# Victarry/Image-Generation-models

Measured on AMD Instinct MI355X. Metric: ddpm_cifar10_32x32_train_images_per_sec, higher is better.
Workload: dtype bf16; 1 GPU; DDPM CIFAR-10 32x32, UNet 128/1-2-4, T=1000 (BASELINE configs[1]): train step B=128/GPU + hipGraph denoise step B=64; per_gpu_batch=128, global_batch=128, parallelism=dp1, step_launch=hipGraph replay, denoise_batch=64, rccl_ranks=1, state_finite=True, matmul=bf16 MFMA, fp32 accumulate

## Files before the change

### image-generation-models_amd/csrc/norm_act.hip

```cpp
#include <stdlib.h>
#include "common.h"

#ifndef MI_GN_UB0
#define MI_GN_UB0 4
#endif
#ifndef MI_GN_PD
#define MI_GN_PD 2
#endif
#ifndef MI_GN_ABL
#define MI_GN_ABL 0
#endif
#ifndef MI_GN_FULL16
#define MI_GN_FULL16 0
#endif
#ifndef MI_GN_WAVES
#define MI_GN_WAVES 4
#endif

namespace {

template <int VEC> struct V;
template <> struct V<4> {
    float v[4];
    __device__ static V load(const float* p) { float4 t = *reinterpret_cast<const float4*>(p); return V{{t.x, t.y, t.z, t.w}}; }
// ... 577 lines not shown
    }
}

template <bool DY16, int LPX, int MAXV>
__global__ __launch_bounds__(256) void chan_ln_bwd_kernel(const LnArgs a) {
    MI_PRIO_UP();
    constexpr int PPW = 64 / LPX;
    __shared__ float red[2][4][LPX * MAXV * 4];
    const int l = threadIdx.x & 63, w = threadIdx.x >> 6, lp = l % LPX;
    const int nq = a.C / 4;
    float4 ag[MAXV], ab[MAXV], gg[MAXV];
#pragma unroll
    for (int k = 0; k < MAXV; ++k) {
        ag[k] = ab[k] = make_float4(0.f, 0.f, 0.f, 0.f);
        int q = lp + LPX * k;
        gg[k] = (q < nq) ? *reinterpret_cast<const float4*>(a.g + 4 * q) : make_float4(0.f, 0.f, 0.f, 0.f);
    }
    for (int m0 = (blockIdx.x * 4 + w) * PPW; m0 < a.M; m0 += gridDim.x * 4 * PPW) {
        const int m = min(m0 + l / LPX, a.M - 1);
        const float live = m0 + l / LPX < a.M ? 1.f : 0.f;
        const float* xp = a.x + (size_t)m * a.ldx;
        float4 c[MAXV], d[MAXV];
        float s = 0.f;
#pragma unroll
        for (int k = 0; k < MAXV; ++k) {
            int q = lp + LPX * k;
            if (q < nq) {
                c[k] = *reinterpret_cast<const float4*>(xp + 4 * q);
                const V<4> dv = vload<4, DY16>(a.dy, (size_t)m * a.lddy + 4 * q);
                d[k] = make_float4(dv.v[0] * live, dv.v[1] * live, dv.v[2] * live, dv.v[3] * live);
                s += c[k].x + c[k].y + c[k].z + c[k].w;
            }
        }
        const float mean = group_sum<LPX>(s) / (float)a.C;
        float s2 = 0.f, sh = 0.f, sS = 0.f;
#pragma unroll
        for (int k = 0; k < MAXV; ++k) {
            if (lp + LPX * k < nq) {
                c[k].x -= mean; c[k].y -= mean; c[k].z -= mean; c[k].w -= mean;
                s2 += c[k].x * c[k].x + c[k].y * c[k].y + c[k].z * c[k].z + c[k].w * c[k].w;
                float h0 = d[k].x * gg[k].x, h1 = d[k].y * gg[k].y, h2 = d[k].z * gg[k].z, h3 = d[k].w * gg[k].w;
                sh += h0 + h1 + h2 + h3;
                sS += h0 * c[k].x + h1 * c[k].y + h2 * c[k].z + h3 * c[k].w;
            }
        }
        const float var = group_sum<LPX>(s2) / (float)a.C;
        const float mh = group_sum<LPX>(sh) / (float)a.C;
        const float S = group_sum<LPX>(sS);
        const float sigma = sqrtf(var);
        const float inv = 1.0f / (sigma + a.eps);
        const float k2 = sigma > 0.f ? inv * inv * S / (sigma * (float)a.C) : 0.f;
        float* op = a.dx + (size_t)m * a.lddx;
        const float* ip = a.dx_in + (size_t)m * a.lddx_in;
#pragma unroll
        for (int k = 0; k < MAXV; ++k) {
            int q = lp + LPX * k;
            if (q < nq) {
                float4 o;
                o.x = inv * (d[k].x * gg[k].x - mh) - k2 * c[k].x;
                o.y = inv * (d[k].y * gg[k].y - mh) - k2 * c[k].y;
                o.z = inv * (d[k].z * gg[k].z - mh) - k2 * c[k].z;
                o.w = inv * (d[k].w * gg[k].w - mh) - k2 * c[k].w;
                if (live != 0.f) {
                    if (a.accumulate) {
                        float4 prev = *reinterpret_cast<const float4*>(ip + 4 * q);
                        o.x += prev.x; o.y += prev.y; o.z += prev.z; o.w += prev.w;
                    }
                    *reinterpret_cast<float4*>(op + 4 * q) = o;
                }
                ag[k].x += d[k].x * c[k].x * inv; ag[k].y += d[k].y * c[k].y * inv;
                ag[k].z += d[k].z * c[k].z * inv; ag[k].w += d[k].w * c[k].w * inv;
                ab[k].x += d[k].x; ab[k].y += d[k].y; ab[k].z += d[k].z; ab[k].w += d[k].w;
            }
        }
    }
#pragma unroll
    for (int k = 0; k < MAXV; ++k) {
        if constexpr (PPW == 2) {
            ag[k].x += __shfl_xor(ag[k].x, 32, 64); ag[k].y += __shfl_xor(ag[k].y, 32, 64); ag[k].z += __shfl_xor(ag[k].z, 32, 64); ag[k].w += __shfl_xor(ag[k].w, 32, 64);
            ab[k].x += __shfl_xor(ab[k].x, 32, 64); ab[k].y += __shfl_xor(ab[k].y, 32, 64); ab[k].z += __shfl_xor(ab[k].z, 32, 64); ab[k].w += __shfl_xor(ab[k].w, 32, 64);
        }
        int q = lp + LPX * k;
        if (q < nq && l < LPX) {
            red[0][w][4 * q + 0] = ag[k].x; red[0][w][4 * q + 1] = ag[k].y; red[0][w][4 * q + 2] = ag[k].z; red[0][w][4 * q + 3] = ag[k].w;
            red[1][w][4 * q + 0] = ab[k].x; red[1][w][4 * q + 1] = ab[k].y; red[1][w][4 * q + 2] = ab[k].z; red[1][w][4 * q + 3] = ab[k].w;
        }
    }
    __syncthreads();
    for (int c = threadIdx.x; c < a.C; c += 256) {
        float v0 = red[0][0][c] + red[0][1][c] + red[0][2][c] + red[0][3][c];
        float v1 = red[1][0][c] + red[1][1][c] + red[1][2][c] + red[1][3][c];
        if (a.part) {
            a.part[(size_t)blockIdx.x * 2 * a.C + c] = v0;
            a.part[(size_t)blockIdx.x * 2 * a.C + a.C + c] = v1;
        } else {
            if (a.dg) atomicAdd(a.dg + c, v0);
            if (a.db) atomicAdd(a.db + c, v1);
        }
    }
}

}

static bool gn_vec8(const GnArgs& a, int io_all16, std::initializer_list<int> lds, std::initializer_list<const void*> ptrs) {
    static const int on = (int)mi_knob("MI_GN_VEC8", 0);
    if (!on || !io_all16 || a.vec8_units <= 4 || a.vec8_units > 8) return false;
    for (int l : lds) if (l % 8) return false;
    for (const void* p : ptrs) if ((uintptr_t)p & 15) return false;
    return true;
}
static bool gn_wide16(const GnArgs& a, std::initializer_list<int> lds, std::initializer_list<const void*> ptrs) {
    if (a.vec8_units <= 8 || a.vec8_units > 16) return false;
    for (int l : lds) if (l % 8) return false;
    for (const void* p : ptrs) if ((uintptr_t)p & 15) return false;
    return true;
}
#define GN_DISPATCH_IO_(KERNEL, IOV, FWD)                                                                 \
    do {                                                                                            \
        dim3 grid(a.N * a.G), blk(256);                                                             \
        if (vec == 8) {                                                                             \
            if (a.vec8_units <= 4) hipLaunchKernelGGL((KERNEL<8, 4, IOV>), grid, blk, 0, st, a);    \
            else hipLaunchKernelGGL((KERNEL<8, 8, IOV>), grid, blk, 0, st, a);                      \
        } else if (vec == 4) {                                                                             \
            if (units <= 4) hipLaunchKernelGGL((KERNEL<4, 4, IOV>), grid, blk, 0, st, a);           \
            else if (units <= 16) hipLaunchKernelGGL((KERNEL<4, 16, IOV>), grid, blk, 0, st, a);    \
            else if (units <= 32 && FWD) hipLaunchKernelGGL((KERNEL<4, 32, IOV>), grid, blk, 0, st, a); \
            else hipLaunchKernelGGL((KERNEL<4, 0, IOV>), grid, blk, 0, st, a);                      \
        } else {                                                                                    \
            if (units <= 16) hipLaunchKernelGGL((KERNEL<1, 16, IOV>), grid, blk, 0, st, a);         \
            else hipLaunchKernelGGL((KERNEL<1, 0, IOV>), grid, blk, 0, st, a);                      \
        }                                                                                           \
    } while (0)
#define GN_DISPATCH_IO(KERNEL, IOV) GN_DISPATCH_IO_(KERNEL, IOV, false)
#define GN_DISPATCH_FWD_IO(KERNEL, IOV) GN_DISPATCH_IO_(KERNEL, IOV, true)
#define GN_DISPATCH(KERNEL) GN_DISPATCH_IO(KERNEL, 0)
#define GN_DISPATCH_BWD16(IOV)                                                                                          \
    do {                                                                                                                \
        const int ppx = 256 / (a.Cg / 4);                                                                               \
        static const int full_on = (int)mi_knob("MI_GN_FULL", 1);                                                       \
        static const int wide_on = (int)mi_knob("MI_GN_WIDE16", 1);                                                     \
        if (full_on && vec == 4 && d->HW == 8 * ppx) hipLaunchKernelGGL((gn_mish_bwd_kernel<4, 8, IOV, true>), dim3(a.N * a.G), dim3(256), 0, st, a); \
        else if (MI_GN_FULL16 && full_on && vec == 4 && d->HW == 16 * ppx) hipLaunchKernelGGL((gn_mish_bwd_kernel<4, 16, IOV, true>), dim3(a.N * a.G), dim3(256), 0, st, a); \
        else if (wide_on && vec == 4 && units > 16 && gn_wide16(a, {d->ldx, lddo, lddx}, {x, dout, dx, gamma, beta}))    \
            hipLaunchKernelGGL((gn_mish_bwd_kernel<8, 16, IOV, false>), dim3(a.N * a.G), dim3(256), 0, st, a);           \
        else GN_DISPATCH_IO(gn_mish_bwd_kernel, IOV);                                                                   \
    } while (0)

extern "C" int mi_gn_mish_fwd(const MiGnDesc* d, const float* x, const float* gamma, const float* beta,
                              const float* temb, int ldt, const float* residual, float* y, float* stats,
                              void* stream) {
    MI_REQUIRE(x && gamma && beta && y, "null argument");
    GnArgs a{};
    int vec, units;
    int rc = gn_prepare(d, a, vec, units);
    MI_REQUIRE(rc == 0, "C/G must be a power of two <= 128 (and 1, 2 or a multiple of 4)");
    MI_REQUIRE(vec == 1 || (d->ldx % 4 == 0 && d->ldy % 4 == 0 && (!residual || d->ldr % 4 == 0)), "ld must be a multiple of 4");
    a.x = x; a.gamma = gamma; a.beta = beta; a.temb = temb; a.ldt = ldt; a.res = residual; a.y = y; a.stats = stats;
    hipStream_t st = (hipStream_t)stream;
    GN_DISPATCH_FWD_IO(gn_mish_fwd_kernel, 0);
    MI_LAUNCH_CHECK();
    return 0;
}

extern "C" int mi_gn_mish_bwd(const MiGnDesc* d, const float* x, const float* stats, const float* gamma,
                              const float* beta, const float* dout, int lddo, float* dx, int lddx,
                              float* dgamma, float* dbeta, float* dtemb, int ldt, float* dbias, void* stream) {
// ... 214 lines not shown
    if (d->HW % (PP * unr)) return 1;
    GnApplyArgs a{};
    a.x = (const uint16_t*)x; a.sums = (const long long*)sums; a.gamma = gamma; a.beta = beta; a.temb = temb; a.res = residual; a.y = y;
    a.y16 = (uint16_t*)y_bf16; a.stats = stats; a.N = d->N; a.HW = d->HW; a.C = C; a.G = G; a.Cg = C / G; a.ldx = d->ldx; a.ldy = d->ldy;
    a.ldr = d->ldr; a.ldt = ldt; a.ldy16 = ldy16; a.eps = d->eps; a.icnt = 1.0 / (MI_GSUM_SCALE * (double)d->HW * (double)(C / G));
    a.chunks = d->HW / (PP * unr);
    const dim3 grid((unsigned)(d->N * a.chunks)), blk(256);
    hipStream_t st = (hipStream_t)stream;
#define GN_APPLY_GO(Y16, RES) do { switch (unr) { \
        case 8: hipLaunchKernelGGL((gn_apply_sums_kernel<Y16, RES, 8>), grid, blk, 0, st, a); break; \
        case 4: hipLaunchKernelGGL((gn_apply_sums_kernel<Y16, RES, 4>), grid, blk, 0, st, a); break; \
        case 2: hipLaunchKernelGGL((gn_apply_sums_kernel<Y16, RES, 2>), grid, blk, 0, st, a); break; \
        default: hipLaunchKernelGGL((gn_apply_sums_kernel<Y16, RES, 1>), grid, blk, 0, st, a); break; } } while (0)
    if (y_is_bf16) GN_APPLY_GO(true, false);
    else if (residual) GN_APPLY_GO(false, true);
    else GN_APPLY_GO(false, false);
#undef GN_APPLY_GO
    MI_LAUNCH_CHECK();
    return 0;
}
extern "C" int mi_gn_mish_bwd_io(const MiGnDesc* d, const void* x, const float* stats, const float* gamma,
                                 const float* beta, const void* dout, int lddo, void* dx, int lddx,
                                 float* dgamma, float* dbeta, float* dtemb, int ldt, float* dbias, int io, void* stream) {
    MI_REQUIRE(x && stats && gamma && beta && dout && dx && !(io & ~7), "bad argument");
    GnArgs a{};
    int vec, units;
    int rc = gn_prepare(d, a, vec, units);
    MI_REQUIRE(rc == 0 && vec >= 4, "bf16 storage needs C/G to be a multiple of 4 (power of two <= 128)");
    MI_REQUIRE(d->ldx % 4 == 0 && lddo % 4 == 0 && lddx % 4 == 0, "ld must be a multiple of 4");
    a.x = (const float*)x; a.stats = const_cast<float*>(stats); a.gamma = gamma; a.beta = beta; a.dout = (const float*)dout; a.lddo = lddo;
    a.dx = (float*)dx; a.lddx = lddx; a.dgamma = dgamma; a.dbeta = dbeta; a.dtemb = dtemb; a.ldt = ldt; a.dbias = dbias;
    if (gn_vec8(a, io & 1, {d->ldx, lddo, lddx}, {x, dout, dx, gamma, beta})) vec = 8;
    hipStream_t st = (hipStream_t)stream;
    switch (io) {
        case 0: GN_DISPATCH_IO(gn_mish_bwd_kernel, 0); break;
        case 1: GN_DISPATCH_BWD16(1); break;
        case 2: GN_DISPATCH_IO(gn_mish_bwd_kernel, 2); break;
        case 3: GN_DISPATCH_BWD16(3); break;
        case 4: GN_DISPATCH_IO(gn_mish_bwd_kernel, 4); break;
        case 5: GN_DISPATCH_BWD16(5); break;
        case 6: GN_DISPATCH_IO(gn_mish_bwd_kernel, 6); break;
        default: GN_DISPATCH_BWD16(7); break;
    }
    MI_LAUNCH_CHECK();
    return 0;
}

static int ln_fwd_go(int M, int C, const float* x, int ldx, const float* g, const float* b, float eps, void* yv, int ldy, int y16, void* stream);
extern "C" int mi_chan_layernorm_fwd(int M, int C, const float* x, int ldx, const float* g, const float* b,
                                     float eps, float* y, int ldy, void* stream) {
    return ln_fwd_go(M, C, x, ldx, g, b, eps, y, ldy, 0, stream);
}
extern "C" int mi_chan_layernorm_fwd_io(int M, int C, const float* x, int ldx, const float* g, const float* b,
                                        float eps, void* y, int ldy, int y16, void* stream) {
    return ln_fwd_go(M, C, x, ldx, g, b, eps, y, ldy, y16, stream);
}
static int ln_fwd_go(int M, int C, const float* x, int ldx, const float* g, const float* b, float eps, void* yv, int ldy, int y16, void* stream) {
    float* y = (float*)yv;
    MI_REQUIRE(M > 0 && C > 0 && C % 4 == 0 && C <= 1024 && ldx % 4 == 0 && ldy % 4 == 0, "C must be a multiple of 4, <= 1024");
    MI_REQUIRE(x && g && b && y, "null argument");
    LnArgs a{};
    a.x = x; a.g = g; a.b = b; a.y = y; a.M = M; a.C = C; a.ldx = ldx; a.ldy = ldy; a.eps = eps;
    const bool half = C <= 128;
    int blocks = (M + (half ? 7 : 3)) / (half ? 8 : 4); if (blocks > 4096) blocks = 4096;
    hipStream_t st = (hipStream_t)stream;
    if (half) { if (y16) hipLaunchKernelGGL((chan_ln_fwd_kernel<true, 32, 1>), dim3(blocks), dim3(256), 0, st, a);
                else     hipLaunchKernelGGL((chan_ln_fwd_kernel<false, 32, 1>), dim3(blocks), dim3(256), 0, st, a); }
    else      { if (y16) hipLaunchKernelGGL((chan_ln_fwd_kernel<true, 64, 4>), dim3(blocks), dim3(256), 0, st, a);
                else     hipLaunchKernelGGL((chan_ln_fwd_kernel<false, 64, 4>), dim3(blocks), dim3(256), 0, st, a); }
    MI_LAUNCH_CHECK();
    return 0;
}

static int ln_bwd_go(int M, int C, const float* x, int ldx, const float* g, float eps, const void* dyv, int lddy, float* dx, int lddx,
                     int accumulate_dx, float* dg, float* db, int dy16, void* stream, float* part = nullptr,
                     const float* dx_in = nullptr, int lddx_in = 0);
static int ln_bwd_blocks(int M, int C) {
    const bool half = C <= 128;
    static const int capenv = (int)mi_knob("MI_LN_BLOCKS", 0);
    const int cap = capenv ? capenv : 512;
    const int blocks = (M + (half ? 7 : 3)) / (half ? 8 : 4);
    return blocks > cap ? cap : blocks;
}
extern "C" int mi_chan_layernorm_bwd(int M, int C, const float* x, int ldx, const float* g, float eps,
                                     const float* dy, int lddy, float* dx, int lddx, int accumulate_dx,
                                     float* dg, float* db, void* stream) {
    return ln_bwd_go(M, C, x, ldx, g, eps, dy, lddy, dx, lddx, accumulate_dx, dg, db, 0, stream);
}
extern "C" int mi_chan_layernorm_bwd_io(int M, int C, const float* x, int ldx, const float* g, float eps,
                                        const void* dy, int lddy, float* dx, int lddx, int accumulate_dx,
                                        float* dg, float* db, int dy16, void* stream) {
    return ln_bwd_go(M, C, x, ldx, g, eps, dy, lddy, dx, lddx, accumulate_dx, dg, db, dy16, stream);
}
extern "C" int mi_chan_layernorm_bwd_part_rows(int M, int C) { return (M > 0 && C > 0) ? ln_bwd_blocks(M, C) : 0; }
extern "C" int mi_chan_layernorm_bwd_part(int M, int C, const float* x, int ldx, const float* g, float eps,
                                          const void* dy, int lddy, float* dx, int lddx, int accumulate_dx,
                                          float* part, int dy16, void* stream) {
    MI_REQUIRE(part, "null argument");
    return ln_bwd_go(M, C, x, ldx, g, eps, dy, lddy, dx, lddx, accumulate_dx, nullptr, nullptr, dy16, stream, part);
}
extern "C" int mi_chan_layernorm_bwd_out(int M, int C, const float* x, int ldx, const float* g, float eps,
                                         const void* dy, int lddy, const float* dx_in, int lddx_in, float* dx_out, int lddx_out,
                                         float* dg, float* db, float* part, int dy16, void* stream) {
    MI_REQUIRE(dx_in && dx_out, "null argument");
    MI_REQUIRE(M > 0 && C > 0 && lddx_in >= C && lddx_out >= C && lddx_in % 4 == 0, "dx_in / dx_out pitch");
    if (dx_in != dx_out) {
        const uintptr_t i0 = (uintptr_t)dx_in, i1 = i0 + ((size_t)(M - 1) * lddx_in + C) * sizeof(float);
        const uintptr_t o0 = (uintptr_t)dx_out, o1 = o0 + ((size_t)(M - 1) * lddx_out + C) * sizeof(float);
        MI_REQUIRE(i1 <= o0 || o1 <= i0, "dx_in and dx_out overlap without being the same tensor");
    } else {
        MI_REQUIRE(lddx_in == lddx_out, "dx_in == dx_out with two pitches");
    }
    return ln_bwd_go(M, C, x, ldx, g, eps, dy, lddy, dx_out, lddx_out, 1, dg, db, dy16, stream, part, dx_in, lddx_in);
}
static int ln_bwd_go(int M, int C, const float* x, int ldx, const float* g, float eps, const void* dyv, int lddy, float* dx, int lddx,
                     int accumulate_dx, float* dg, float* db, int dy16, void* stream, float* part, const float* dx_in, int lddx_in) {
    const float* dy = (const float*)dyv;
    MI_REQUIRE(M > 0 && C > 0 && C % 4 == 0 && C <= 1024 && ldx % 4 == 0 && lddy % 4 == 0 && lddx % 4 == 0, "C must be a multiple of 4, <= 1024");
    MI_REQUIRE(x && g && dy && dx, "null argument");
    LnArgs a{};
    a.x = x; a.g = g; a.dy = dy; a.dx = dx; a.dg = dg; a.db = db; a.M = M; a.C = C; a.ldx = ldx; a.lddy = lddy;
    a.lddx = lddx; a.accumulate = accumulate_dx; a.eps = eps; a.part = part;
    a.dx_in = dx_in ? dx_in : dx; a.lddx_in = dx_in ? lddx_in : lddx;
    const bool half = C <= 128;
    const int blocks = ln_bwd_blocks(M, C);
    hipStream_t st = (hipStream_t)stream;
    if (half) { if (dy16) hipLaunchKernelGGL((chan_ln_bwd_kernel<true, 32, 1>), dim3(blocks), dim3(256), 0, st, a);
                else      hipLaunchKernelGGL((chan_ln_bwd_kernel<false, 32, 1>), dim3(blocks), dim3(256), 0, st, a); }
    else      { if (dy16) hipLaunchKernelGGL((chan_ln_bwd_kernel<true, 64, 4>), dim3(blocks), dim3(256), 0, st, a);
                else      hipLaunchKernelGGL((chan_ln_bwd_kernel<false, 64, 4>), dim3(blocks), dim3(256), 0, st, a); }
    MI_LAUNCH_CHECK();
    return 0;
}
```

### image-generation-models_amd/src/ops/lib.py

```python
from __future__ import annotations

import ctypes as C
import os

_PKG_ROOT = os.path.dirname(os.path.dirname(os.path.dirname(os.path.abspath(__file__))))
_LIB = None


def library_path() -> str:
    return os.environ.get("MI_DDPM_LIB", os.path.join(_PKG_ROOT, "lib", "libmi_ddpm.so"))


class MiConvDesc(C.Structure):
    _fields_ = [(n, C.c_int) for n in (
        "N", "IH", "IW", "OH", "OW", "K", "Nc", "KH", "KW", "stride", "pad", "transposed", "w_kn", "mode",
        "K1", "ldx", "ldx2", "ldy", "ldr", "accumulate")]


class MiWgradDesc(C.Structure):
    _fields_ = [(n, C.c_int) for n in (
        "N", "GH", "GW", "DH", "DW", "Ci", "Cj", "KH", "KW", "stride", "pad", "gather_i", "mode", "I1",
        "ldp", "ldp2", "ldq")]


# ... 77 lines not shown
    "mi_conv3x3_pw_supported": [C.POINTER(MiConvDesc)],
    "mi_conv3x3_pw_tile": [C.POINTER(MiConvDesc)],
    "mi_debug_conv_pw_tile": [_I],
    "mi_debug_conv_pw_auto256": [_I],
    "mi_debug_conv1x1_pw_nloop": [_I],
    "mi_conv3x3_pw_f32_tile": [C.POINTER(MiConvDesc)],
    "mi_conv3x3_pw_f32": [C.POINTER(MiConvDesc), _P, _P, _P, _P, _P, _P, _P],
    "mi_conv1x1_pw_x32_supported": [C.POINTER(MiConvDesc)],
    "mi_conv1x1_pw_x32": [C.POINTER(MiConvDesc), _P, _P, _P, _P, _P, _P, _I, _P],
    "mi_conv_pw_set_splitk_workspace": [_P, C.c_size_t],
    "mi_conv3x3_pw_splitk": [C.POINTER(MiConvDesc), _I, _I],
    "mi_debug_conv_pw_splitk": [_I],
    "mi_ln_conv1x1_pw_supported": [C.POINTER(MiConvDesc)],
    "mi_ln_conv1x1_pw": [C.POINTER(MiConvDesc), _P, _P, _P, C.c_float, _P, _P, _P, _P],
    "mi_ln_conv1x1_pw_dual": [C.POINTER(MiConvDesc), _P, _P, _P, C.c_float, _P, _P, _P, _P, _I, _P],
    "mi_conv1x1_pw_f32_supported": [C.POINTER(MiConvDesc)],
    "mi_conv1x1_pw_f32": [C.POINTER(MiConvDesc), _P, _P, _P, _P, _P, _P, _P],
    "mi_pack_weights_f32frag": [_I, _P, _I, _P, _P, _P, _P],
    "mi_conv3x3_pw_x32_supported": [C.POINTER(MiConvDesc)],
    "mi_conv3x3_pw_x32_tile": [C.POINTER(MiConvDesc)],
    "mi_conv3x3_pw_x32": [C.POINTER(MiConvDesc), _P, _P, _P, _P, _P, _P, _I, _P, _P],
    "mi_conv3x3_pw": [C.POINTER(MiConvDesc), _P, _P, _P, _P, _P, _P, _I, _P],
    "mi_conv3x3_pw_gn_mish_supported": [C.POINTER(MiConvDesc)],
    "mi_conv1x1_pw_supported": [C.POINTER(MiConvDesc)],
    "mi_conv1x1_pw": [C.POINTER(MiConvDesc), _P, _P, _P, _P, _P, _P, _I, _P, _I, _P],
    "mi_conv3x3_pw_gnsums": [C.POINTER(MiConvDesc), _P, _P, _P, _P, _P, _P, _I, _P, _P],
    "mi_conv3x3_pw_gn_mish": [C.POINTER(MiConvDesc), _P, _P, _P, _P, _P, _I, _P],
    "mi_conv3x3_pw_gn_mish_sums": [C.POINTER(MiConvDesc), _P, _P, _P, _P, _P, _I, _I, _F, _P, _P, _P, _I, _P],
    "mi_conv3x3_pw_x32_gn_mish_supported": [C.POINTER(MiConvDesc)],
    "mi_conv3x3_pw_x32_gn_mish_tile": [C.POINTER(MiConvDesc)],
    "mi_conv3x3_pw_gn_mish_tile": [C.POINTER(MiConvDesc)],
    "mi_conv3x3_pw_x32_gn_mish": [C.POINTER(MiConvDesc), _P, _P, _P, _P, _P, _I, _P],
    "mi_conv3x3_pw_x32_gn_mish_sums": [C.POINTER(MiConvDesc), _P, _P, _P, _P, _P, _I, _I, _F, _P, _P, _P, _I, _P],
    "mi_gn_stats_coef": [C.POINTER(MiGnDesc), _P, _P, _P, _P, _I, _P, _P, _I, _P],
    "mi_conv3x3_gn_mish_supported": [C.POINTER(MiConvDesc)],
    "mi_conv3x3_gn_mish_tile": [C.POINTER(MiConvDesc), C.POINTER(C.c_int), C.POINTER(C.c_int)],
    "mi_conv3x3_gn_mish": [C.POINTER(MiConvDesc), _P, _P, _P, _P, _P, _I, _P],
    "mi_conv3x3_small_cin_fwd": [_I, _I, _I, _I, _I, _P, _I, _P, _P, _P, _I, _P],
    "mi_conv3x3_small_cin_wgrad": [_I, _I, _I, _I, _I, _P, _I, _P, _I, _P, _P],
    "mi_conv1x1_small_cout": [_I, _I, _I, _I, _P, _I, _P, _I, _P, _P, _P, _I, _I, _P],
    "mi_conv1x1_small_cout_ws": [_I, _I, _I, _I, _P, _I, _P, _I, _P, _P, _P, _I, _I, _P, _Z, _P],
    "mi_conv1x1_small_cout_io": [_I, _I, _I, _I, _P, _I, _P, _I, _P, _P, _P, _I, _I, _I, _P, _Z, _P],
    "mi_linattn_fold_fwd": [_I, _I, _I, _P, _P, _I, _P, _P],
    "mi_conv1x1_pw_batched": [C.POINTER(MiConvDesc), _P, _P, _I, _P, _P, _P, _I, _P, _I, _P],
    "mi_conv1x1_small_cout_bwd": [_I, _I, _I, _P, _I, _I, _P, _I, _P, _P, _P, _I, _I, _I, _P, C.c_size_t, _P],
    "mi_conv1x1_small_cout_gn_supported": [_I, _I, _I],
    "mi_conv1x1_small_cout_gn_fwd": [_I, _I, _I, _I, _P, _I, _P, _P, _P, _I, C.c_float, _P, _P, _P, _I, _P],
    "mi_conv_small_cin_fwd_dual_supported": [_I, _I, _I, _I, _I, _I],
    "mi_conv_small_cin_fwd_dual_chores": [_I, _I, _I, _I, _I, _P, _I, _P, _P, _P, _I, _I, _P, _P, _P, _I, _P, C.c_size_t, _P, _P, _P, _I, _I, _P],
    "mi_conv_small_cin_fwd_dual": [_I, _I, _I, _I, _I, _P, _I, _P, _P, _P, _I, _I, _P, _P, _P, _I, _P],
    "mi_conv_small_cin_fwd_io": [_I, _I, _I, _I, _I, _I, _P, _I, _P, _P, _P, _I, _I, _P],
    "mi_conv_small_cin_wgrad_io": [_I, _I, _I, _I, _I, _I, _P, _I, _P, _I, _I, _P, _P, _Z, _P],
    "mi_conv_small_cin_bf16_supported": [_I, _I, _I, _I, _I, _I, _I],
    "mi_conv_small_cin_fwd": [_I, _I, _I, _I, _I, _I, _P, _I, _P, _P, _P, _I, _P],
    "mi_conv_small_cin_wgrad": [_I, _I, _I, _I, _I, _I, _P, _I, _P, _I, _P, _P, _Z, _P],
    "mi_conv_wgrad": [C.POINTER(MiWgradDesc), _P, _P, _P, _P, _P],
    "mi_conv3x3_wgrad": [C.POINTER(MiWgradDesc), _P, _P, _P, _P, _P],
    "mi_conv3x3_wgrad_supported": [C.POINTER(MiWgradDesc)],
    "mi_conv3x3_wgrad_ws": [C.POINTER(MiWgradDesc), _P, _P, _P, _P, _P, _Z, _P],
    "mi_conv3x3_wgrad_bias": [C.POINTER(MiWgradDesc), _P, _P, _P, _P, _P, _P, _Z, _P],
    "mi_colsum": [_I, _I, _P, _I, _P, _P],
    "mi_colsum_ordered": [_I, _I, _P, _I, _P, _P, _Z, _P],
    "mi_conv_wgrad_slabs": [C.POINTER(MiWgradDesc), _P, _P, _P, _P, _P, _Z, _P],
    "mi_gn_mish_fwd": [C.POINTER(MiGnDesc), _P, _P, _P, _P, _I, _P, _P, _P, _P],
    "mi_gn_mish_bwd": [C.POINTER(MiGnDesc), _P, _P, _P, _P, _P, _I, _P, _I, _P, _P, _P, _I, _P, _P],
    "mi_chan_layernorm_fwd": [_I, _I, _P, _I, _P, _P, _F, _P, _I, _P],
    "mi_chan_layernorm_bwd": [_I, _I, _P, _I, _P, _F, _P, _I, _P, _I, _I, _P, _P, _P],
    "mi_linattn_fwd": [_I, _I, _I, _P, _P, _P, _P, _P],
    "mi_linattn_bwd": [_I, _I, _I, _P, _P, _P, _P, _P, _P],
    "mi_vq_partials": [_I],
    "mi_vq_nearest_fwd": [_I, _I, _I, _P, _I, _P, _P, _P, _I, _P, _P],
    "mi_vq_bwd": [_I, _I, _I, _P, _I, _P, _P, _F, _F, _P, _P, _I, _I, _P, _P],
    "mi_vq_scatter_rows": [_I, _I, _I, _P, _I, _P, _P, _P],
    "mi_small_gemm": [_I, _I, _I, _I, _I, _P, _I, _P, _I, _P, _P, _I, _I, _I, _P],
    "mi_small_gemm_supported": [_I, _I, _I, _I, _I, _I, _I],
    "mi_linattn_fwd_io": [_I, _I, _I, _P, _P, _P, _P, _I, _P],
    "mi_linattn_bwd_io": [_I, _I, _I, _P, _P, _P, _P, _P, _I, _P],
    "mi_linattn_fwd_ws": [_I, _I, _I, _P, _P, _P, _P, _I, _P, _Z, _P],
    "mi_linattn_bwd_ws": [_I, _I, _I, _P, _P, _P, _P, _P, _I, _P, _Z, _P],
    "mi_chan_layernorm_fwd_io": [_I, _I, _P, _I, _P, _P, _F, _P, _I, _I, _P],
    "mi_chan_layernorm_bwd_io": [_I, _I, _P, _I, _P, _F, _P, _I, _P, _I, _I, _P, _P, _I, _P],
    "mi_chan_layernorm_bwd_part": [_I, _I, _P, _I, _P, _F, _P, _I, _P, _I, _I, _P, _I, _P],
    "mi_chan_layernorm_bwd_out": [_I, _I, _P, _I, _P, _F, _P, _I, _P, _I, _P, _I, _P, _P, _P, _I, _P],
    "mi_rowsum_batch": [_I, _P, _P],
    "mi_f32_to_bf16_colsum_part": [_Z, _I, _P, _I, _P, _I, _P, _Z, C.POINTER(C.c_int), _P],
    "mi_time_embed": [_I, _I, _P, _P, _P],
    "mi_sample_norm_supported": [_I, _I, _I],
    "mi_sample_norm_fwd": [_I, _I, _I, _P, _P, _P, _P, _P, _F, _P],
    "mi_sample_norm_bwd": [_I, _I, _I, _P, _P, _P, _P, _P, _P, _P, _P, _P],
    "mi_sample_norm_bwd2": [_I, _I, _I, _P, _P, _P, _P, _P, _P, _P, _P, _P],
    "mi_leaky_relu_fwd": [_Z, _P, _P, _F, _P],
    "mi_leaky_relu_bwd": [_Z, _P, _P, _P, _F, _P],
    "mi_tanh_fwd": [_Z, _P, _P, _P],
    "mi_tanh_bwd": [_Z, _P, _P, _P, _P],
    "mi_lerp_rows": [_I, _Z, _P, _P, _P, _P, _P],
    "mi_gp_penalty": [_I, _Z, _P, _P, _P, _F, _P, _P],
    "mi_batchnorm_workspace": [_I],
    "mi_batchnorm_fwd": [_I, _I, _P, _P, _P, _P, _P, _P, _P, _P, _F, _F, _I, _P, _P],
    "mi_batchnorm_bwd": [_I, _I, _P, _P, _P, _P, _P, _P, _P, _P, _P, _P],
    "mi_vae_latent_fwd": [_I, _I, _P, _I, _P, _P, _P, _P],
    "mi_vae_latent_bwd": [_I, _I, _P, _I, _P, _P, _F, _P, _P, _I, _P],
    "mi_cvae_pack_input": [_I, _I, _I, _I, _P, _P, _P, _I, _P],
    "mi_cvae_latent_fwd": [_I, _I, _I, _P, _I, _P, _P, _P, _P, _P, _P],
    "mi_cvae_latent_bwd": [_I, _I, _I, _P, _I, _P, _P, _P, _I, _F, _P, _P, _P, _P],
    "mi_latent_disc_supported": [_I, _I, _I],
    "mi_latent_disc_fwd": [_I, _I, _I, _P, _I, _P, _I, _P, _P, _P, _I, _F, _F, _P, _P, _P, _P, _P, _P],
    "mi_latent_disc_bwd": [_I, _I, _I, _P, _I, _P, _I, _P, _P, _P, _I, _F, _P, _P, _P, _F, _I, _P, _I, _F, _I, _P],
    "mi_latent_disc_ln_supported": [_I, _I, _I, _I],
    "mi_latent_disc_ln_fwd": [_I, _I, _I, _I, _P, _I, _P, _I, _P, _I, _F, _F, _P, _P, _P],
    "mi_latent_disc_ln_bwd": [_I, _I, _I, _I, _P, _I, _P, _I, _P, _I, _F, _F, _F, _F, _P, _P, _P, _F, _I, _P, _I, _F, _I, _P],
    "mi_bn_seg_rows_per_workgroup": [_I, _I],
    "mi_bn_seg_fwd": [_I, _I, _I, _P, _P, _P, _P, _P, _P, _P, _P, _F, _F, _I, _I, _F, _P, _P],
    "mi_bn_seg_bwd": [_I, _I, _I, _P, _P, _P, _P, _P, _P, _P, _P, _P, _I, _I, _F, _P, _P],
    "mi_adv_loss": [_I, _I, _I, C.POINTER(C.c_int), _F, _P, _I, _P, _P, _P, _I, _P],
    "mi_info_latent": [_I, _I, _I, _I, _I, _P, _P, _I, _P, _I, _P, _I, _P],
    "mi_info_head_supported": [_I, _I, _I, _I, _I, _I, _I],
    "mi_info_head_fwd": [_I, _I, _I, _I, _P, _I, _P, _I, _I, _F, _I, _I, _I, _P, _P, _I, _F, _P, _P, _P, _P, _P, _P, _P, _P],
    "mi_info_head_bwd": [_I, _I, _I, _I, _I, _P, _I, _P, _P, _P, _P, _P, _I, _P, _P, _P],
    "mi_age_moments_supported": [_I, _I, _I],
    "mi_age_image_mse": [_I, _I, _I, _P, _I, _P, _P, _P, _F, _P, _P],
    "mi_age_moments_fwd": [_I, _I, _I, _P, _I, _I, _P, _P, _I, _I, _I, _P, _I, _P, _P, _P, _P, _P],
    "mi_age_moments_bwd": [_I, _I, _I, _P, _I, _P, _P, _P, _F, _F, _I, _I, _F, _F, _P, _I, _P, _P, _I, _P, _I, _P],
    "mi_rmsprop_step": [_Z, _P, _P, _P, _F, _F, _F, _F, _P],
    "mi_clamp_inplace": [_Z, _P, _F, _F, _P],
    "mi_adam_tick": [_P, _P],
    "mi_adam_step_dev": [_Z, _P, _P, _P, _P, _P, C.c_double, C.c_double, _F, _F, _P],
    "mi_relu_fwd": [_Z, _P, _P, _P],
    "mi_relu_bwd": [_Z, _P, _P, _P, _I, _P],
    "mi_mish_fwd": [_Z, _P, _P, _P],
    "mi_mish_bwd": [_Z, _P, _P, _P, _P],
    "mi_nchw_to_nhwc": [_I, _I, _I, _P, _P, _I, _P],
    "mi_nhwc_to_nchw": [_I, _I, _I, _P, _I, _P, _P],
    "mi_q_sample": [_I, _I, _I, _P, _P, _P, _P, _P, _P, _I, _P, _P],
    "mi_eps_loss": [_I, _I, _I, _P, _I, _P, _I, _P, _P, _F, _P],
    "mi_p_sample_update": [_I, _I, _I, _P, _P, _I, _P, _P, _P, _P, _P, _P, _P, _I, _P, _P, _I, _P],
    "mi_adam_step": [_Z, _P, _P, _P, _P, _F, _F, _F, _F, _F, _F, _F, _P],
    "mi_adam_step_c": [_Z, _P, _P, _P, _P, _F, _F, _F, _F, _F, _F, _F, _F, _P],
    "mi_axpby": [_Z, _F, _P, _I, _P, _P],
    "mi_axpby2d": [_I, _I, _F, _P, _I, _I, _P, _I, _P],
    "mi_gather_rows": [_I, _I, _P, _P, _P, _P],
    "mi_u8_gather_normalize": [_I, _I, _I, _I, _P, _P, _P, _I, _P, _P],
    "mi_scale_by_device_scalar": [_I, _I, _P, _I, _P, _P],
    "mi_pcnn_conv_supported": [C.POINTER(MiPcnnConvDesc)],
    "mi_pcnn_conv": [C.POINTER(MiPcnnConvDesc), _P, _P, _P, _P, _P, _P, _P, _P, _P, _P, _P, _P],
    "mi_pcnn_wgrad_supported": [C.POINTER(MiPcnnConvDesc)],
    "mi_pcnn_wgrad": [C.POINTER(MiPcnnConvDesc), _P, _P, _I, _P, _P],
    "mi_pcnn_colsum": [_I, _I, _P, _I, _P, _P, _P],
    "mi_pcnn_gate_bwd_supported": [_I],
    "mi_pcnn_gate_bwd": [_I, _I, _I, _I, _P, _I, _P, _I, _P, _I, _P, _I, _P, _P],
    "mi_pcnn_small_mm": [_I, _I, _I, _P, _I, _I, _P, _I, _I, _P, _I, _I, _P],
    "mi_pcnn_cond_rows": [_I, _I, _I, _P, _P, _P, _I, _P],
    "mi_pcnn_cond_wgrad": [_I, _I, _I, _P, _P, _I, _P, _P],
    "mi_pcnn_head_supported": [_I, _I],
    "mi_pcnn_head_partials": [_I, _I, _I],
    "mi_pcnn_head_fwd": [_I, _I, _I, _I, _P, _I, _P, _P, _P, _I, _P, _P, _P, _P],
    "mi_pcnn_head_dlogits": [_I, _I, _I, _I, _P, _I, _P, _P, _P, _I, _P, _P, _P, _P],
    "mi_pcnn_sample_supported": [_I, _I, _I],
    "mi_pcnn_sample_step": [_I, _I, _I, _I, _I, _P, _I, _P, _P, _P, _P, _P, _P, _I, _I, _P],
    "mi_pcnn_zero": [_P, _Z, _P],
    "mi_made_supported": [_I, _I, _I],
    "mi_made_linear": [_I, _I, _I, _I, _P, _I, _P, _P, _P, _P, _I, _P, _I, _P],
    "mi_made_dgrad": [_I, _I, _I, _I, _P, C.c_longlong, _P, _P, _P, _P, _I, _P, _P, _I, _P],
    "mi_made_wgrad": [_I, _I, _I, _I, _P, C.c_longlong, _P, _I, _P, _P, _P, _P, _P],
    "mi_made_head_partials": [_I, _I],
    "mi_made_head_fwd": [_I, _I, _I, _I, _P, _I, _P, _P, _P, _P, _P, _I, _P, _P, _P, _P],
    "mi_made_head_dlogits": [_I, _I, _I, _I, _P, _I, _P, _P, _P, _P, _P, _I, _P, _P, _P, _P],
# ... 62 lines not shown
```

### include/mi_ddpm.h

```cpp
#ifndef MI_DDPM_H
#define MI_DDPM_H
#include <stddef.h>
#include <stdint.h>

#ifdef __cplusplus
extern "C" {
#endif

#define MI_ABI_VERSION 4
#define MI_MODE_FP32 0
#define MI_MODE_BF16 1

int mi_abi_version(void);
const char* mi_last_error(void);

typedef struct MiConvDesc {
    int N;
    int IH, IW;
    int OH, OW;
    int K;
    int Nc;
    int KH, KW, stride, pad;
    int transposed;
    int w_kn;
// ... 177 lines not shown
int mi_debug_wgrad_tr_blocks(int blocks);

int mi_conv_s2_wgrad_tr_supported(const MiWgradDesc* d);
size_t mi_conv_s2_wgrad_tr_batch_workspace(int n, const MiWgradDesc* descs);
int mi_conv_s2_wgrad_tr_batch(int n, const MiWgradDesc* descs, const void* const* P, const void* const* Q, float* const* dW,
                              void* workspace, size_t ws_bytes, void* stream);
int mi_debug_wgrad_s2_tr_phase(int phase);

#define MI_WGRAD_STORE 1u
int mi_conv3x3_wgrad_tr_batch_ex(int n, const MiWgradDesc* descs, const void* const* P, const void* const* P2,
                                 const void* const* Q, float* const* dW, void* workspace, size_t ws_bytes, void* stream, unsigned flags);
int mi_conv1x1_wgrad_tr_batch_ex(int n, const MiWgradDesc* descs, const int* q_is_fp32, const void* const* P,
                                 const void* const* P2, const void* const* Q, float* const* dW, float* const* dbias,
                                 void* workspace, size_t ws_bytes, void* stream, unsigned flags);
int mi_conv_s2_wgrad_tr_batch_ex(int n, const MiWgradDesc* descs, const void* const* P, const void* const* Q, float* const* dW,
                                 void* workspace, size_t ws_bytes, void* stream, unsigned flags);

int mi_conv_s2_wgrad_f32_supported(const MiWgradDesc* d);
size_t mi_conv_s2_wgrad_f32_workspace(const MiWgradDesc* d);
int mi_conv_s2_wgrad_f32(const MiWgradDesc* d, const float* P, const float* Q, float* dW, void* workspace, size_t ws_bytes, void* stream);
int mi_debug_spin(int blocks, int usec, float* buf, size_t per_wg_floats, int mode, void* stream);
int mi_debug_clock_probe(int blocks, int usec, unsigned long long* out3, void* stream);

size_t mi_f32_to_bf16_colsum_workspace(size_t M, int C);
int mi_f32_to_bf16_colsum(size_t M, int C, const float* x, int ldx, void* y_bf16, int ldy, float* colsum, void* workspace,
                          size_t ws_bytes, void* stream);
int mi_f32_to_bf16_colsum_part(size_t M, int C, const float* x, int ldx, void* y_bf16, int ldy, float* part, size_t part_bytes,
                               int* rows, void* stream);
int mi_colsum(int M, int C, const float* x, int ld, float* out, void* stream);
size_t mi_colsum_ordered_workspace(int M, int C);
int mi_colsum_ordered(int M, int C, const float* x, int ld, float* out, void* ws, size_t ws_bytes, void* stream);
size_t mi_conv_wgrad_slabs_workspace(const MiWgradDesc* d);
int mi_conv_wgrad_slabs(const MiWgradDesc* d, const float* P, const float* P2, const float* Q, float* dW, void* ws, size_t ws_bytes,
                        void* stream);
#define MI_ROWSUM_MAX 16
typedef struct { const float* src; float* dst; int rows, cols, ld, pad_; } MiRowSum;
int mi_rowsum_batch(int n, const MiRowSum* items, void* stream);
int mi_zero_ranges(const long long* table_dev, int n, float* base, void* stream);

typedef struct MiGnDesc {
    int N, HW, C, G;
    float eps;
    int ldx, ldy, ldr;
} MiGnDesc;

int mi_gn_mish_fwd(const MiGnDesc* d, const float* x, const float* gamma, const float* beta,
                   const float* temb, int ldt, const float* residual, float* y, float* stats,
                   void* stream);
int mi_gn_mish_bwd(const MiGnDesc* d, const float* x, const float* stats, const float* gamma,
                   const float* beta, const float* dout, int lddo, float* dx, int lddx,
                   float* dgamma, float* dbeta, float* dtemb, int ldt, float* dbias,
                   void* stream);

int mi_gn_mish_fwd_io(const MiGnDesc* d, const void* x, const float* gamma, const float* beta, const float* temb,
                      int ldt, const float* residual, void* y, float* stats, int io, void* stream);
int mi_gn_mish_fwd_dual(const MiGnDesc* d, const void* x, const float* gamma, const float* beta,
                        const float* temb, int ldt, const float* residual, void* y, void* y16, int ldy16,
                        float* stats, int io, void* stream);
int mi_gn_mish_apply_sums(const MiGnDesc* d, const void* x, const void* sums, const float* gamma, const float* beta, const float* temb,
                          int ldt, const float* residual, void* y, int y_is_bf16, void* y_bf16, int ldy16, float* stats, void* stream);
int mi_gn_stats_coef(const MiGnDesc* d, const void* x, const float* gamma, const float* beta, const float* temb, int ldt,
                     float* stats, float* coef, int x_is_bf16, void* stream);
int mi_gn_mish_bwd_io(const MiGnDesc* d, const void* x, const float* stats, const float* gamma, const float* beta,
                      const void* dout, int lddo, void* dx, int lddx, float* dgamma, float* dbeta, float* dtemb,
                      int ldt, float* dbias, int io, void* stream);

int mi_chan_layernorm_fwd(int M, int C, const float* x, int ldx, const float* g, const float* b,
                          float eps, float* y, int ldy, void* stream);
int mi_chan_layernorm_bwd(int M, int C, const float* x, int ldx, const float* g, float eps,
                          const float* dy, int lddy, float* dx, int lddx, int accumulate_dx,
                          float* dg, float* db, void* stream);
int mi_chan_layernorm_fwd_io(int M, int C, const float* x, int ldx, const float* g, const float* b,
                             float eps, void* y, int ldy, int y16, void* stream);
int mi_chan_layernorm_bwd_io(int M, int C, const float* x, int ldx, const float* g, float eps,
                             const void* dy, int lddy, float* dx, int lddx, int accumulate_dx,
                             float* dg, float* db, int dy16, void* stream);
int mi_chan_layernorm_bwd_part_rows(int M, int C);
int mi_chan_layernorm_bwd_part(int M, int C, const float* x, int ldx, const float* g, float eps,
                               const void* dy, int lddy, float* dx, int lddx, int accumulate_dx,
                               float* part, int dy16, void* stream);
int mi_chan_layernorm_bwd_out(int M, int C, const float* x, int ldx, const float* g, float eps,
                              const void* dy, int lddy, const float* dx_in, int lddx_in, float* dx_out, int lddx_out,
                              float* dg, float* db, float* part, int dy16, void* stream);

int mi_linattn_fwd(int B, int n, int heads, const float* qkv, float* out, float* ctx,
                   float* kstat, void* stream);
int mi_linattn_bwd(int B, int n, int heads, const float* qkv, const float* ctx,
                   const float* kstat, const float* dout, float* dqkv, void* stream);
int mi_linattn_fwd_io(int B, int n, int heads, const void* qkv, void* out, float* ctx, float* kstat, int b16,
                      void* stream);
int mi_linattn_bwd_io(int B, int n, int heads, const void* qkv, const float* ctx, const float* kstat,
                      const void* dout, void* dqkv, int b16, void* stream);
size_t mi_linattn_workspace(int B, int n, int heads);
int mi_linattn_fwd_ws(int B, int n, int heads, const void* qkv, void* out, float* ctx, float* kstat, int b16,
                      void* workspace, size_t ws_bytes, void* stream);
int mi_linattn_bwd_ws(int B, int n, int heads, const void* qkv, const float* ctx, const float* kstat,
                      const void* dout, void* dqkv, int b16, void* workspace, size_t ws_bytes, void* stream);

int mi_small_gemm(int ta, int tb, int I, int J, int K, const float* A, int lda, const float* B, int ldb,
                  const float* bias, float* C, int ldc, int accumulate, int allow_split, void* stream);
int mi_small_gemm_supported(int ta, int tb, int I, int J, int K, int lda, int ldb);

int mi_vq_partials(int M);
int mi_vq_nearest_fwd(int M, int D, int K, const float* z, int ldz, const float* codebook, int* idx, float* zq, int ldq,
                      float* loss_partial, void* stream);
int mi_vq_bwd(int M, int D, int K, const float* z, int ldz, const float* codebook, const int* idx, float g_vq, float g_commit,
              const float* g_dev, float* dz, int lddz, int accumulate_dz, float* dcodebook, void* stream);
int mi_vq_scatter_rows(int M, int D, int K, const float* src, int ld, const int* idx, float* table, void* stream);

int mi_sample_norm_supported(int N, int P, int C);
int mi_sample_norm_fwd(int N, int P, int C, const float* x, const float* gamma, const float* beta, float* y, float* stats, float eps,
                       void* stream);
int mi_sample_norm_bwd(int N, int P, int C, const float* x, const float* stats, const float* gamma, const float* dy, const float* extra_dx,
                       float* dx, float* dgamma, float* dbeta, void* stream);
int mi_sample_norm_bwd2(int N, int P, int C, const float* x, const float* stats, const float* gamma, const float* dy, const float* u,
                        float* adj_dy, float* adj_x, float* dgamma, void* stream);
int mi_leaky_relu_fwd(size_t n, const float* x, float* y, float slope, void* stream);
int mi_leaky_relu_bwd(size_t n, const float* y, const float* dy, float* dx, float slope, void* stream);
int mi_tanh_fwd(size_t n, const float* x, float* y, void* stream);
int mi_tanh_bwd(size_t n, const float* y, const float* dy, float* dx, void* stream);
int mi_lerp_rows(int N, size_t per, const float* a, const float* b, const float* e, float* out, void* stream);
int mi_gp_penalty(int N, size_t per, const float* g, float* penalty, float* u, float scale, const float* scale_dev, void* stream);

int mi_batchnorm_workspace(int C);
int mi_batchnorm_fwd(int M, int C, const float* x, const float* gamma, const float* beta, float* y, float* mean, float* rstd,
                     float* running_mean, float* running_var, float momentum, float eps, int training, void* ws, void* stream);
int mi_batchnorm_bwd(int M, int C, const float* x, const float* mean, const float* rstd, const float* gamma, const float* dy,
                     float* dx, float* dgamma, float* dbeta, void* ws, void* stream);
int mi_vae_latent_fwd(int N, int L, const float* h, int ldh, const float* eps, float* z, float* kld, void* stream);
int mi_vae_latent_bwd(int N, int L, const float* h, int ldh, const float* eps, const float* dz, float g_kld, const float* g_dev,
                      float* dh, int lddh, void* stream);

int mi_cvae_pack_input(int N, int C, int HW, int ncls, const float* x_nchw, const int64_t* labels, float* y_nhwc, int ld, void* stream);
int mi_cvae_latent_fwd(int N, int L, int ncls, const float* h, int ldh, const float* eps, const int64_t* labels, const float* E,
                       float* zc, float* kld, void* stream);
int mi_cvae_latent_bwd(int N, int L, int ncls, const float* h, int ldh, const float* eps, const int64_t* labels, const float* dzc,
                       int lddzc, float g_kld, const float* g_dev, float* dh, float* dE, void* stream);

#define MI_LATENT_DISC_NMAX 1024
int mi_latent_disc_supported(int N, int L, int H);
size_t mi_latent_disc_tape_floats(int N);
size_t mi_latent_disc_workspace_floats(int N);
int mi_latent_disc_fwd(int N, int L, int H, const float* z, int ldz, const float* h, int ldh, const float* eps, const int64_t* perm,
                       const float* const* params, int training, float target, float momentum, float* running_mean, float* running_var,
                       int64_t* num_batches_tracked, float* tape, float* out3, void* stream);
int mi_latent_disc_bwd(int N, int L, int H, const float* z, int ldz, const float* h, int ldh, const float* eps, const int64_t* perm,
                       const float* const* params, int training, float target, const float* tape, float* workspace, float* const* grads,
                       float param_scale, int accumulate_params, float* dz, int lddz, float dz_scale, int accumulate_dz, void* stream);

#define MI_LATENT_DISC_LN_NMAX 65536
int mi_latent_disc_ln_supported(int N0, int N1, int L, int H);
size_t mi_latent_disc_ln_tape_floats(int N);
size_t mi_latent_disc_ln_workspace_floats(int N);
int mi_latent_disc_ln_fwd(int N0, int N1, int L, int H, const float* x0, int ld0, const float* x1, int ld1, const float* const* params,
                          int loss_mode, float target0, float target1, float* tape, float* out5, void* stream);
int mi_latent_disc_ln_bwd(int N0, int N1, int L, int H, const float* x0, int ld0, const float* x1, int ld1, const float* const* params,
                          int loss_mode, float target0, float target1, float c0, float c1, const float* tape, float* workspace,
                          float* const* grads, float param_scale, int accumulate_params, float* dx0, int lddx, float dx_scale,
                          int accumulate_dx, void* stream);

size_t mi_bn_seg_workspace(int S, int M, int C);
int mi_bn_seg_rows_per_workgroup(int M, int C);
int mi_bn_seg_fwd(int S, int M, int C, const float* x, const float* gamma, const float* beta, float* y, float* mean, float* rstd,
                  float* running_mean, float* running_var, float momentum, float eps, int training, int act, float slope, void* ws,
                  void* stream);
int mi_bn_seg_bwd(int S, int M, int C, const float* x, const float* mean, const float* rstd, const float* gamma, const float* y,
// ... 128 lines not shown
```

Baseline: 27710 images/s.

## Add software-pipelined channel LayerNorm backward kernel with batched row loads

Adds a new channel-LayerNorm backward kernel that issues loads for several row groups (U=2 or 4) before computing any of them, so memory latency overlaps instead of serializing per row. It specializes on compile-time C (128/256/512) and on whether dx is accumulated, and keeps bf16 dy as raw packed words unpacked in registers. The kernel is used by default when alignment and C conditions hold, and falls back to the old kernel otherwise. In exchange it uses more registers per thread, which may lower occupancy, and the different FMA ordering may change rounding slightly.

```diff
diff --git a/image-generation-models_amd/csrc/norm_act.hip b/image-generation-models_amd/csrc/norm_act.hip
--- a/image-generation-models_amd/csrc/norm_act.hip
+++ b/image-generation-models_amd/csrc/norm_act.hip
@@ -683,6 +683,128 @@
         }
         int q = lp + LPX * k;
         if (q < nq && l < LPX) {
+            red[0][w][4 * q + 0] = ag[k].x; red[0][w][4 * q + 1] = ag[k].y; red[0][w][4 * q + 2] = ag[k].z; red[0][w][4 * q + 3] = ag[k].w;
+            red[1][w][4 * q + 0] = ab[k].x; red[1][w][4 * q + 1] = ab[k].y; red[1][w][4 * q + 2] = ab[k].z; red[1][w][4 * q + 3] = ab[k].w;
+        }
+    }
+    __syncthreads();
+    for (int c = threadIdx.x; c < a.C; c += 256) {
+        float v0 = red[0][0][c] + red[0][1][c] + red[0][2][c] + red[0][3][c];
+        float v1 = red[1][0][c] + red[1][1][c] + red[1][2][c] + red[1][3][c];
+        if (a.part) {
+            a.part[(size_t)blockIdx.x * 2 * a.C + c] = v0;
+            a.part[(size_t)blockIdx.x * 2 * a.C + a.C + c] = v1;
+        } else {
+            if (a.dg) atomicAdd(a.dg + c, v0);
+            if (a.db) atomicAdd(a.db + c, v1);
+        }
+    }
+}
+
+typedef uint32_t u32x2 __attribute__((ext_vector_type(2)));
+template <bool DY16> struct LnDyRaw { typedef f32x4 type; };
+template <> struct LnDyRaw<true> { typedef u32x2 type; };
+
+template <bool DY16, int LPX, int NV, bool ACC> struct LnGroup {
+    typedef typename LnDyRaw<DY16>::type dy_t;
+    f32x4 x[NV], prev[NV]; dy_t dy[NV];
+    int m; float live;
+    __device__ __forceinline__ void load(const LnArgs& a, int m0, int l, int lp) {
+        m = min(m0 + l / LPX, a.M - 1);
+        live = m0 + l / LPX < a.M ? 1.f : 0.f;
+        const float* xp = a.x + (size_t)m * a.ldx;
+        const float* ip = a.dx_in + (size_t)m * a.lddx_in;
+#pragma unroll
+        for (int k = 0; k < NV; ++k) {
+            const int q = lp + LPX * k;
+            x[k] = *reinterpret_cast<const f32x4*>(xp + 4 * q);
+            if constexpr (DY16) dy[k] = *reinterpret_cast<const u32x2*>(reinterpret_cast<const uint16_t*>(a.dy) + (size_t)m * a.lddy + 4 * q);
+            else dy[k] = *reinterpret_cast<const f32x4*>(a.dy + (size_t)m * a.lddy + 4 * q);
+            if constexpr (ACC) prev[k] = *reinterpret_cast<const f32x4*>(ip + 4 * q);
+        }
+    }
+    __device__ __forceinline__ void finish(const LnArgs& a, int lp, const f32x4 (&gg)[NV], f32x4 (&ag)[NV], f32x4 (&ab)[NV]) {
+#pragma clang fp contract(off)
+        f32x4 c[NV], d[NV];
+        float s = 0.f;
+#pragma unroll
+        for (int k = 0; k < NV; ++k) {
+            c[k] = x[k];
+            f32x4 dv;
+            if constexpr (DY16) dv = f32x4{__uint_as_float(dy[k].x << 16), __uint_as_float(dy[k].x & 0xffff0000u),
+                                           __uint_as_float(dy[k].y << 16), __uint_as_float(dy[k].y & 0xffff0000u)};
+            else dv = dy[k];
+            d[k] = f32x4{dv.x * live, dv.y * live, dv.z * live, dv.w * live};
+            s += c[k].x + c[k].y + c[k].z + c[k].w;
+        }
+        const float mean = group_sum<LPX>(s) / (float)a.C;
+        float s2 = 0.f, sh = 0.f, sS = 0.f;
+#pragma unroll
+        for (int k = 0; k < NV; ++k) {
+            c[k].x -= mean; c[k].y -= mean; c[k].z -= mean; c[k].w -= mean;
+            s2 += c[k].x * c[k].x + c[k].y * c[k].y + c[k].z * c[k].z + c[k].w * c[k].w;
+            float h0 = d[k].x * gg[k].x, h1 = d[k].y * gg[k].y, h2 = d[k].z * gg[k].z, h3 = d[k].w * gg[k].w;
+            sh += h0 + h1 + h2 + h3;
+            sS += h0 * c[k].x + h1 * c[k].y + h2 * c[k].z + h3 * c[k].w;
+        }
+        const float var = group_sum<LPX>(s2) / (float)a.C;
+        const float mh = group_sum<LPX>(sh) / (float)a.C;
+        const float S = group_sum<LPX>(sS);
+        const float sigma = sqrtf(var);
+        const float inv = 1.0f / (sigma + a.eps);
+        const float k2 = sigma > 0.f ? inv * inv * S / (sigma * (float)a.C) : 0.f;
+        float* op = a.dx + (size_t)m * a.lddx;
+#pragma unroll
+        for (int k = 0; k < NV; ++k) {
+            const int q = lp + LPX * k;
+            f32x4 o;
+            o.x = __builtin_fmaf(inv, __builtin_fmaf(d[k].x, gg[k].x, -mh), -(k2 * c[k].x));
+            o.y = __builtin_fmaf(inv, __builtin_fmaf(d[k].y, gg[k].y, -mh), -(k2 * c[k].y));
+            o.z = __builtin_fmaf(inv, __builtin_fmaf(d[k].z, gg[k].z, -mh), -(k2 * c[k].z));
+            o.w = __builtin_fmaf(inv, __builtin_fmaf(d[k].w, gg[k].w, -mh), -(k2 * c[k].w));
+            if constexpr (ACC) { o.x += prev[k].x; o.y += prev[k].y; o.z += prev[k].z; o.w += prev[k].w; }
+            if (live != 0.f) *reinterpret_cast<f32x4*>(op + 4 * q) = o;
+            ag[k].x = __builtin_fmaf(d[k].x * c[k].x, inv, ag[k].x); ag[k].y = __builtin_fmaf(d[k].y * c[k].y, inv, ag[k].y);
+            ag[k].z = __builtin_fmaf(d[k].z * c[k].z, inv, ag[k].z); ag[k].w = __builtin_fmaf(d[k].w * c[k].w, inv, ag[k].w);
+            ab[k].x += d[k].x; ab[k].y += d[k].y; ab[k].z += d[k].z; ab[k].w += d[k].w;
+        }
+    }
+};
+
+template <bool DY16, int LPX, int NV, bool ACC, int U>
+__global__ __launch_bounds__(256) void chan_ln_bwd_pipe_kernel(const LnArgs a) {
+    MI_PRIO_UP();
+    constexpr int PPW = 64 / LPX;
+    __shared__ float red[2][4][LPX * NV * 4];
+    const int l = threadIdx.x & 63, w = __builtin_amdgcn_readfirstlane(threadIdx.x >> 6), lp = l % LPX;
+    f32x4 ag[NV], ab[NV], gg[NV];
+#pragma unroll
+    for (int k = 0; k < NV; ++k) {
+        ag[k] = ab[k] = f32x4{0.f, 0.f, 0.f, 0.f};
+        gg[k] = *reinterpret_cast<const f32x4*>(a.g + 4 * (lp + LPX * k));
+    }
+    const int step = gridDim.x * 4 * PPW;
+    int m0 = (blockIdx.x * 4 + w) * PPW;
+    for (; a.M - m0 > (U - 1) * step; m0 += U * step) {
+        LnGroup<DY16, LPX, NV, ACC> grp[U];
+#pragma unroll
+        for (int u = 0; u < U; ++u) grp[u].load(a, m0 + u * step, l, lp);
+#pragma unroll
+        for (int u = 0; u < U; ++u) grp[u].finish(a, lp, gg, ag, ab);
+    }
+    for (; m0 < a.M; m0 += step) {
+        LnGroup<DY16, LPX, NV, ACC> grp;
+        grp.load(a, m0, l, lp);
+        grp.finish(a, lp, gg, ag, ab);
+    }
+#pragma unroll
+    for (int k = 0; k < NV; ++k) {
+        if constexpr (PPW == 2) {
+            ag[k].x += __shfl_xor(ag[k].x, 32, 64); ag[k].y += __shfl_xor(ag[k].y, 32, 64); ag[k].z += __shfl_xor(ag[k].z, 32, 64); ag[k].w += __shfl_xor(ag[k].w, 32, 64);
+            ab[k].x += __shfl_xor(ab[k].x, 32, 64); ab[k].y += __shfl_xor(ab[k].y, 32, 64); ab[k].z += __shfl_xor(ab[k].z, 32, 64); ab[k].w += __shfl_xor(ab[k].w, 32, 64);
+        }
+        const int q = lp + LPX * k;
+        if (l < LPX) {
             red[0][w][4 * q + 0] = ag[k].x; red[0][w][4 * q + 1] = ag[k].y; red[0][w][4 * q + 2] = ag[k].z; red[0][w][4 * q + 3] = ag[k].w;
             red[1][w][4 * q + 0] = ab[k].x; red[1][w][4 * q + 1] = ab[k].y; red[1][w][4 * q + 2] = ab[k].z; red[1][w][4 * q + 3] = ab[k].w;
         }
@@ -1063,6 +1185,19 @@
     const int blocks = (M + (half ? 7 : 3)) / (half ? 8 : 4);
     return blocks > cap ? cap : blocks;
 }
+static int g_ln_pipe = 1;
+extern "C" int mi_debug_ln_bwd_pipeline(int on) {
+    const int was = g_ln_pipe;
+    g_ln_pipe = on != 0;
+    return was;
+}
+extern "C" int mi_chan_layernorm_bwd_pipelined(int C, const void* x, const void* dy, const void* dx, const void* dx_in, int ldx, int lddy,
+                                               int lddx, int lddx_in, int dy16) {
+    if (!g_ln_pipe || (C != 128 && C != 256 && C != 512)) return 0;
+    if (ldx % 4 || lddy % 4 || lddx % 4 || (dx_in && lddx_in % 4)) return 0;
+    if (((uintptr_t)x | (uintptr_t)dx | (uintptr_t)dx_in) & 15) return 0;
+    return ((uintptr_t)dy & (dy16 ? 7 : 15)) == 0;
+}
 extern "C" int mi_chan_layernorm_bwd(int M, int C, const float* x, int ldx, const float* g, float eps,
                                      const float* dy, int lddy, float* dx, int lddx, int accumulate_dx,
                                      float* dg, float* db, void* stream) {
@@ -1106,6 +1241,19 @@
     const bool half = C <= 128;
     const int blocks = ln_bwd_blocks(M, C);
     hipStream_t st = (hipStream_t)stream;
+    if (mi_chan_layernorm_bwd_pipelined(C, x, dy, dx, accumulate_dx ? a.dx_in : nullptr, ldx, lddy, lddx, a.lddx_in, dy16)) {
+#define LN_PIPE_GO(DY16, LPX, NV, U)                                                                                                   \
+        do {                                                                                                                           \
+            if (accumulate_dx) hipLaunchKernelGGL((chan_ln_bwd_pipe_kernel<DY16, LPX, NV, true, U>), dim3(blocks), dim3(256), 0, st, a);  \
+            else               hipLaunchKernelGGL((chan_ln_bwd_pipe_kernel<DY16, LPX, NV, false, U>), dim3(blocks), dim3(256), 0, st, a); \
+        } while (0)
+        if (C == 128)      { if (dy16) LN_PIPE_GO(true, 32, 1, 4); else LN_PIPE_GO(false, 32, 1, 4); }
+        else if (C == 256) { if (dy16) LN_PIPE_GO(true, 64, 1, 4); else LN_PIPE_GO(false, 64, 1, 4); }
+        else               { if (dy16) LN_PIPE_GO(true, 64, 2, 2); else LN_PIPE_GO(false, 64, 2, 2); }
+#undef LN_PIPE_GO
+        MI_LAUNCH_CHECK();
+        return 0;
+    }
     if (half) { if (dy16) hipLaunchKernelGGL((chan_ln_bwd_kernel<true, 32, 1>), dim3(blocks), dim3(256), 0, st, a);
                 else      hipLaunchKernelGGL((chan_ln_bwd_kernel<false, 32, 1>), dim3(blocks), dim3(256), 0, st, a); }
     else      { if (dy16) hipLaunchKernelGGL((chan_ln_bwd_kernel<true, 64, 4>), dim3(blocks), dim3(256), 0, st, a);
diff --git a/image-generation-models_amd/src/ops/lib.py b/image-generation-models_amd/src/ops/lib.py
--- a/image-generation-models_amd/src/ops/lib.py
+++ b/image-generation-models_amd/src/ops/lib.py
@@ -183,6 +183,8 @@
     "mi_chan_layernorm_bwd_io": [_I, _I, _P, _I, _P, _F, _P, _I, _P, _I, _I, _P, _P, _I, _P],
     "mi_chan_layernorm_bwd_part": [_I, _I, _P, _I, _P, _F, _P, _I, _P, _I, _I, _P, _I, _P],
     "mi_chan_layernorm_bwd_out": [_I, _I, _P, _I, _P, _F, _P, _I, _P, _I, _P, _I, _P, _P, _P, _I, _P],
+    "mi_chan_layernorm_bwd_pipelined": [_I, _P, _P, _P, _P, _I, _I, _I, _I, _I],
+    "mi_debug_ln_bwd_pipeline": [_I],
     "mi_rowsum_batch": [_I, _P, _P],
     "mi_f32_to_bf16_colsum_part": [_Z, _I, _P, _I, _P, _I, _P, _Z, C.POINTER(C.c_int), _P],
     "mi_time_embed": [_I, _I, _P, _P, _P],
diff --git a/include/mi_ddpm.h b/include/mi_ddpm.h
--- a/include/mi_ddpm.h
+++ b/include/mi_ddpm.h
@@ -283,6 +283,9 @@
 int mi_chan_layernorm_bwd_out(int M, int C, const float* x, int ldx, const float* g, float eps,
                               const void* dy, int lddy, const float* dx_in, int lddx_in, float* dx_out, int lddx_out,
                               float* dg, float* db, float* part, int dy16, void* stream);
+int mi_chan_layernorm_bwd_pipelined(int C, const void* x, const void* dy, const void* dx, const void* dx_in, int ldx, int lddy,
+                                    int lddx, int lddx_in, int dy16);
+int mi_debug_ln_bwd_pipeline(int on);
 
 int mi_linattn_fwd(int B, int n, int heads, const float* qkv, float* out, float* ctx,
                    float* kstat, void* stream);
```

New measurement: 27990 images/s, median of 6. 1.0% higher.
